# sudo-monkey/fabric-token-sdk

Hardware: AMD Instinct MI355X
Metric: zkatdlog transfer proofs verified/sec (node) + BN254 G1 MSM 2^20 latency (higher is better)
Workload: dtype u32 (Fp/Fr Montgomery); 1 GPU; batch verify 4096 zkatdlog transfers per GPU per step (BASELINE configs[1]); 1-GPU job of 2260992 transfers sharded by tx (configs[3]); batch_per_gpu=4096, device_pass=8192, pp=b=100,e=2, fexp=exact, parallelism=tx-sharded x1

## Files before the change

fabric-token-sdk_amd/csrc/dev/jobs.h:

```cpp
#pragma once
#include "fp29.h"
#include "fp_wide.h"
#include "glv.h"
#include "pairing.h"
#include "sha256.h"

namespace fts {

static constexpr uint32_t NONE = 0xFFFFFFFFu;

struct G1Dev {
  uint32_t x[8], y[8];
};
struct G2Dev {
  uint32_t x0[8], x1[8], y0[8], y1[8];
};
struct F12Dev {
  uint32_t w[96];
};

enum G1Base : uint8_t { G1B_PED0 = 0, G1B_PED1, G1B_PED2, G1B_PEDGEN, G1B_GEN, G1B_COUNT };
static constexpr uint32_t G1B_SIG0 = G1B_COUNT;
static constexpr uint32_t G1B_SIG_MAX_DIGITS = (255 - G1B_SIG0) / 2;
enum G2Base : uint8_t { G2B_PK0 = 0, G2B_PK1, G2B_PK2, G2B_Q, G2B_COUNT };
// ... 27 lines not shown
enum ScalOp : uint32_t { SOP_MUL = 0, SOP_MULK = 1, SOP_SUM = 2, SOP_MADD = 3, SOP_MULK64 = 4 };
struct ScalJob {
  uint32_t op, a, b, out, c;
};

struct VTerm {
  uint32_t pt;
  uint32_t w_lo, w_hi;
  uint32_t flags;
};
static constexpr uint32_t VT_HORNER = 1;
static constexpr uint32_t VT_NEG = 2;

struct G1Job {
  uint32_t fscal[3];
  uint8_t fbase[3];
  uint8_t nfix;
  uint32_t vstart, vcount;
  uint32_t vscal;
  uint32_t vneg;
  uint32_t out;
  uint32_t bytes;
  uint32_t b64;
};

struct G2Job {
  uint32_t fscal[3];
  uint8_t fbase[3];
  uint8_t nfix;
  uint32_t out;
};

struct PairJob {
  uint32_t p1;
  uint32_t p2;
  uint32_t q2;
  uint32_t bytes;
  uint32_t p3;
};

struct Seg {
  uint32_t off, len;
};

struct HashJob {
  uint32_t seg_start, seg_count;
  uint32_t expect;
// ... 607 lines not shown
}

FTS_HD void job_g1(const G1Job& j, const VTerm* vterms, const G1Dev* pts, const uint32_t (*scal)[8],
                   const G1Dev* tab, G1Dev* g1out, uint8_t* arena) {
  g1j acc = jac_inf<fp>();
  if (j.vscal != NONE) {
    g1j V = g1_var_point(j, vterms, pts);
    if (j.vneg) V = jac_neg(V);
    G1Dev loc[16];
    if (!is_zero(V.z)) acc = g1_mul_glv16_iso(g1a{V.x, V.y, false}, V.z, scal[j.vscal], loc, 1);
  }
  for (int f = 0; f < j.nfix; f++) acc = g1_fixed_acc(acc, tab, j.fbase[f], scal[j.fscal[f]]);
  g1a r = jac_to_aff(acc);
  G1Dev d;
  g1_store(d, r);
  g1out[j.out] = d;
  g1_emit_bytes(j, r, arena);
}

FTS_HD void job_g1_part(const G1Job* jobs, uint32_t n, uint32_t i, const VTerm* vterms, const G1Dev* pts,
                        const uint32_t (*scal)[8], const G1Dev* tab, G1JDev* part, G1Dev* vtab) {
  uint32_t f = i / n, jb = i - f * n;
  const G1Job& j = jobs[jb];
  g1j acc = jac_inf<fp>();
  if (f < 3) {
    if (f < j.nfix) acc = g1_fixed_acc(acc, tab, j.fbase[f], scal[j.fscal[f]]);
  } else if (j.vscal != NONE) {
    g1j V = g1_var_point(j, vterms, pts);
    if (j.vneg) V = jac_neg(V);
#if FTS_G1_VAR_W == 16
#if defined(__HIP_DEVICE_COMPILE__)
    G1Dev* tb = vtab + jb;
    const size_t st = n;
#else
    G1Dev loc[16];
    G1Dev* tb = vtab ? vtab + jb : loc;
    const size_t st = vtab ? n : 1;
#endif
    if (!is_zero(V.z)) acc = g1_mul_glv16_iso(g1a{V.x, V.y, false}, V.z, scal[j.vscal], tb, st);
#else
    acc = g1_mul_glv(jac_to_aff(V), scal[j.vscal]);
#endif
  }
  g1j_store(part[i], acc);
}

FTS_HD g1j job_g1_sum_parts(const G1Job& j, uint32_t jb, uint32_t n, const G1JDev* part) {
  g1j acc = g1j_load(part[3 * (size_t)n + jb]);
  for (uint32_t f = 0; f < 3; f++)
    if (f < j.nfix) acc = jac_add(acc, g1j_load(part[(size_t)f * n + jb]));
  return acc;
}

FTS_HD void job_g1_finish(const G1Job& j, const g1j& acc, const fp& zi, G1Dev* g1out, uint8_t* arena) {
  g1a r;
  r.inf = is_zero(acc.z);
  fp zi2 = sqr(zi);
  r.x = r.inf ? fe_zero<ModP>() : acc.x * zi2;
  r.y = r.inf ? fe_zero<ModP>() : acc.y * zi2 * zi;
  G1Dev d;
  g1_store(d, r);
  g1out[j.out] = d;
  g1_emit_bytes(j, r, arena);
}

FTS_HD void g1_pnorm(const g1j& acc, const fp& inv, G1Dev& out) {
  fp z2 = sqr(acc.z);
  G1Dev d;
  g1_store(d, g1a{acc.x * z2 * inv, sqr(z2) * inv, false});
  out = d;
}
// ... 333 lines not shown
```

fabric-token-sdk_amd/csrc/host/planner.cpp:

```cpp
#include "planner.h"

#include <math.h>
#include <string.h>

#include <algorithm>
#include <atomic>
#include <condition_variable>
#include <mutex>
#include <thread>
#include <type_traits>

#include "gojson.h"

namespace ftsh {

static const JField LEAVES_F[] = {{nullptr, JF_STRUCT, nullptr}};
static const JField SIGPROOF_F[] = {{"Signature", JF_STRUCT, LEAVES_F}, {nullptr, JF_STRUCT, nullptr}};
static const JField MP_F[] = {{"SignatureProofs", JF_SLICE, SIGPROOF_F}, {nullptr, JF_STRUCT, nullptr}};
static const JField RANGE_F[] = {{"EqualityProofs", JF_STRUCT, LEAVES_F},
                                 {"MembershipProofs", JF_SLICE, MP_F},
                                 {nullptr, JF_STRUCT, nullptr}};
static const JField RPP_F[] = {{"SignedValues", JF_SLICE, LEAVES_F}, {nullptr, JF_STRUCT, nullptr}};
static const JField PP_F[] = {{"RangeProofParams", JF_STRUCT, RPP_F}, {nullptr, JF_STRUCT, nullptr}};

void Plan::clear() {
  rnd.clear();
  sc1.clear();
  sc_post.clear();
  emit.clear();
  b64.clear();
  cp.clear();
  cp2.clear();
  out.clear();
  out_off.clear();
  item_off.clear();
  dev_pools = false;
  arena_len = out_len = 0;
  wire.clear();
  arena.clear();
  dec.clear();
  zr.clear();
  sc.clear();
  sclist.clear();
  vt.clear();
  g1.clear();
  g1p.clear();
  g2.clear();
  pr.clear();
  seg.clear();
  hpre.clear();
  hmain.clear();
  ck.clear();
  tx.clear();
  n_pts = n_scal = n_g1out = n_g2out = 0;
}

namespace {

// ... 242 lines not shown
    pl.seg.push_back({off, len});
    return (uint32_t)pl.seg.size() - 1;
  }
  uint32_t g1job(std::initializer_list<std::pair<uint8_t, uint32_t>> fixed, const std::vector<VTerm>& var,
                 uint32_t vscal, uint32_t bytes, bool feeds_pairing = false) {
    G1Job j;
    memset(&j, 0, sizeof(j));
    j.nfix = 0;
    for (auto& f : fixed) {
      j.fbase[j.nfix] = f.first;
      j.fscal[j.nfix] = f.second;
      j.nfix++;
    }
    j.vstart = (uint32_t)pl.vt.size();
    j.vcount = (uint32_t)var.size();
    pl.vt.insert(pl.vt.end(), var.begin(), var.end());
    j.vscal = vscal;
    j.vneg = 1;
    j.out = pl.n_g1out++;
    j.bytes = bytes;
    j.b64 = NONE;
    (feeds_pairing ? pl.g1p : pl.g1).push_back(j);
    return j.out;
  }
  uint32_t dbg_scal() { return pp.debug_challenges ? pl.n_scal++ : NONE; }
  static VTerm vterm(uint32_t pt, uint64_t w = 1) {
    VTerm v;
    v.pt = pt;
    v.w_lo = (uint32_t)w;
    v.w_hi = (uint32_t)(w >> 32);
    v.flags = 0;
    return v;
  }

  void begin_tx(uint8_t mode) {
    tc.wf_start = (uint32_t)pl.ck.size();
    ncheck[0] = ncheck[1] = 0;
    part = 0;
    tc.mode = mode;
  }
  void begin_range() {
    tc.wf_count = ncheck[0];
    tc.rg_start = (uint32_t)pl.ck.size();
    part = 1;
  }
  void end_tx() {
// ... 126 lines not shown
  }
  if (s_type == NONE) s_type = scalar(type);
  if (s_sum == NONE) s_sum = scalar(sum);
  if (s_chal == NONE) s_chal = scalar(chal);
  uint32_t s_tn = pl.n_scal++;
  pl.sc.push_back({SOP_MULK, s_type, n, s_tn});
  uint32_t s_bf[64];
  std::vector<uint32_t> bfi(n), vai(n);
  for (uint32_t i = 0; i < n; i++) {
    vai[i] = scalar(vals[i]);
    bfi[i] = scalar(bfs[i]);
  }
  (void)s_bf;
  uint32_t s_bfsum = pl.n_scal++;
  pl.sc.push_back({SOP_SUM, (uint32_t)pl.sclist.size(), n, s_bfsum});
  pl.sclist.insert(pl.sclist.end(), bfi.begin(), bfi.end());
  std::vector<VTerm> all;
  for (uint32_t i = 0; i < n; i++) {
    g1job({{G1B_PED0, s_type}, {G1B_PED1, vai[i]}, {G1B_PED2, bfi[i]}}, {vterm(tok_pt + i)}, s_chal,
          wfout_bytes + 64 * i);
    all.push_back(vterm(tok_pt + i));
  }
  g1job({{G1B_PED0, s_tn}, {G1B_PED1, s_sum}, {G1B_PED2, s_bfsum}}, all, s_chal, wfout_bytes + 64 * n);
  return true;
}

void Builder::decode_range(Doc& doc, RangeDoc& r) {
  int64_t top = doc.top();
  r.chal = doc.elem(doc.f(top, "Challenge"));
  bool isnil;
  int64_t eq = doc.obj(doc.f(top, "EqualityProofs"), isnil);
  r.eq_nil = isnil;
  if (!isnil) {
    r.eq_type = doc.elem(doc.f(eq, "Type"));
    r.eq_val = doc.list(doc.f(eq, "Value"));
    r.eq_tbf = doc.list(doc.f(eq, "TokenBlindingFactor"));
    r.eq_cbf = doc.list(doc.f(eq, "CommitmentBlindingFactor"));
  }
  int64_t mps = doc.f(top, "MembershipProofs");
  if (mps >= 0 && doc.d.at((uint32_t)mps).type != J_NULL) {
    if (doc.d.at((uint32_t)mps).type != J_ARR) {
      doc.err = true;
      return;
    }
    uint32_t n = doc.d.len((uint32_t)mps);
    r.mps.resize(n);
// ... 533 lines not shown
    s.fn = &f;
    s.n = n;
    s.next.store(0);
    s.active = (size_t)nthreads_;
    s.gen++;
  }
  s.cv.notify_all();
  for (size_t i; (i = s.next.fetch_add(1)) < n;) f(i);
  std::unique_lock<std::mutex> lk(s.mu);
  s.done_cv.wait(lk, [&]() { return s.active == 0; });
}

namespace {

constexpr size_t SEC_ALIGN = 256;
constexpr size_t IDX_LIMIT = (size_t)1 << 31;

size_t elem_size(int s) {
  switch (s) {
    case PS_WIRE: case PS_ARENA: case PS_OUT: return 1;
    case PS_DEC: return sizeof(DecodeJob);
    case PS_ZR: return sizeof(ZrJob);
    case PS_SC: case PS_SC1: case PS_SCPOST: return sizeof(ScalJob);
    case PS_SCLIST: return sizeof(uint32_t);
    case PS_VT: return sizeof(VTerm);
    case PS_G1: case PS_G1P: return sizeof(G1Job);
    case PS_G2: return sizeof(G2Job);
    case PS_PR: return sizeof(PairJob);
    case PS_SEG: return sizeof(Seg);
    case PS_HPRE: case PS_HMAIN: return sizeof(HashJob);
    case PS_CK: return sizeof(Check);
    case PS_TX: return sizeof(TxChecks);
    case PS_RND: return sizeof(RandJob);
    case PS_EMIT: return sizeof(EmitJob);
    case PS_B64: return sizeof(B64Job);
    case PS_CP: case PS_CP2: return sizeof(CopyJob);
  }
  return 1;
}

size_t piece_count(const Plan& p, int s) {
  switch (s) {
    case PS_WIRE: return p.wire.size();
    case PS_ARENA: return p.dev_pools ? p.arena_len : p.arena.size();
    case PS_DEC: return p.dec.size();
    case PS_ZR: return p.zr.size();
    case PS_SC: return p.sc.size();
// ... 55 lines not shown
    j.out += o_scal;
    return j;
  };
  const int scs[3] = {PS_SC, PS_SC1, PS_SCPOST};
  const std::vector<ScalJob>* scv[3] = {&b.sc, &b.sc1, &b.sc_post};
  for (int k = 0; k < 3; k++) {
    ScalJob* d = reinterpret_cast<ScalJob*>(dst[scs[k]]) + o.sec[scs[k]];
    for (const ScalJob& j : *scv[k]) *d++ = rel_sc(j);
  }
  uint32_t* sl = reinterpret_cast<uint32_t*>(dst[PS_SCLIST]) + o.sec[PS_SCLIST];
  for (uint32_t v : b.sclist) *sl++ = v + o_scal;
  VTerm* vt = reinterpret_cast<VTerm*>(dst[PS_VT]) + o.sec[PS_VT];
  for (VTerm v : b.vt) {
    v.pt += o_pts;
    *vt++ = v;
  }
  for (int side = 0; side < 2; side++) {
    int sec = side ? PS_G1P : PS_G1;
    G1Job* d = reinterpret_cast<G1Job*>(dst[sec]) + o.sec[sec];
    for (G1Job j : (side ? b.g1p : b.g1)) {
      for (int k = 0; k < j.nfix; k++) j.fscal[k] += o_scal;
      j.vstart += o_vt;
      j.vscal = rel(j.vscal, o_scal);
      j.out += o_g1;
      j.bytes = rel(j.bytes, o_arena);
      j.b64 = rel(j.b64, o_arena);
      *d++ = j;
    }
  }
  G2Job* g2 = reinterpret_cast<G2Job*>(dst[PS_G2]) + o.sec[PS_G2];
  for (G2Job j : b.g2) {
    for (int k = 0; k < j.nfix; k++) j.fscal[k] += o_scal;
    j.out += o_g2;
    *g2++ = j;
  }
  PairJob* pr = reinterpret_cast<PairJob*>(dst[PS_PR]) + o.sec[PS_PR];
  for (PairJob j : b.pr) {
    j.p1 += o_g1;
    j.p2 += p2_g1out ? o_g1 : o_pts;
    j.q2 = rel(j.q2, o_g2);
    j.p3 = rel(j.p3, o_g1);
    j.bytes += o_arena;
    *pr++ = j;
  }
  Seg* sg = reinterpret_cast<Seg*>(dst[PS_SEG]) + o.sec[PS_SEG];
  for (Seg s : b.seg) {
// ... 42 lines not shown
  }
  B64Job* bj = reinterpret_cast<B64Job*>(dst[PS_B64]) + o.sec[PS_B64];
  for (B64Job j : b.b64) {
    j.src += o_arena;
    j.dst += o_out;
    *bj++ = j;
  }
  const int cps[2] = {PS_CP, PS_CP2};
  const std::vector<CopyJob>* cpv[2] = {&b.cp, &b.cp2};
  for (int k = 0; k < 2; k++) {
    CopyJob* d = reinterpret_cast<CopyJob*>(dst[cps[k]]) + o.sec[cps[k]];
    for (CopyJob j : *cpv[k]) {
      j.src += o_wire;
      j.dst += j.to_out ? o_out : o_arena;
      *d++ = j;
    }
  }
}

void relocate_piece(const Plan& b, const PieceBase& o, const FlatPlan& fp, uint8_t* blob) {
  uint8_t* dst[PS_COUNT];
  for (int s = 0; s < PS_COUNT; s++) dst[s] = blob + fp.off[s];
  relocate_into(b, o, fp.p2_g1out, false, dst);
}

}

std::string flat_layout(const PlanWork& w, bool p2_g1out, FlatPlan& fp) {
  fp.p2_g1out = p2_g1out;
  fp.base.assign(w.used, PieceBase{});
  fp.out_off.clear();
  fp.item_off.clear();
  fp.n_items = 0;
  size_t cur[PS_COUNT] = {};
  cur[PS_ARENA] = C_SIZE;
  uint64_t pts = 0, scal = 0, g1 = 0, g2 = 0;
  for (size_t k = 0; k < w.used; k++) {
    const Plan& p = w.pieces[k];
    PieceBase& b = fp.base[k];
    cur[PS_WIRE] = (cur[PS_WIRE] + 15) & ~(size_t)15;
    cur[PS_ARENA] = (cur[PS_ARENA] + 15) & ~(size_t)15;
    for (int s = 0; s < PS_COUNT; s++) {
      b.sec[s] = cur[s];
      cur[s] += piece_count(p, s);
    }
    b.pts = (uint32_t)pts;
    b.scal = (uint32_t)scal;
    b.g1out = (uint32_t)g1;
    b.g2out = (uint32_t)g2;
    pts += p.n_pts;
    scal += p.n_scal;
    g1 += p.n_g1out;
    g2 += p.n_g2out;
    for (uint32_t v : p.out_off) fp.out_off.push_back((uint32_t)(v + b.sec[PS_OUT]));
    for (uint32_t v : p.item_off) fp.item_off.push_back((uint32_t)(v + b.sec[PS_ARENA]));
    fp.n_items += p.tx.size();
  }
  if (!fp.out_off.empty() || cur[PS_OUT]) fp.out_off.push_back((uint32_t)cur[PS_OUT]);
  for (int s = 0; s < PS_COUNT; s++)
    if (cur[s] >= IDX_LIMIT) return "batch too large for 32-bit job indices (split it into smaller batches)";
  if (pts >= IDX_LIMIT || scal >= IDX_LIMIT || g1 >= IDX_LIMIT || g2 >= IDX_LIMIT)
    return "batch too large for 32-bit job indices (split it into smaller batches)";
  fp.n_pts = (uint32_t)pts;
  fp.n_scal = (uint32_t)scal;
  fp.n_g1out = (uint32_t)g1;
  fp.n_g2out = (uint32_t)g2;
  fp.dev_pools = w.used > 0;
  for (size_t k = 0; k < w.used; k++) fp.dev_pools = fp.dev_pools && w.pieces[k].dev_pools;
  int order[PS_COUNT], no = 0;
  for (int s = 0; s < PS_COUNT; s++)
    if (!fp.dev_pools || (s != PS_ARENA && s != PS_OUT)) order[no++] = s;
  if (fp.dev_pools) {
    order[no++] = PS_ARENA;
    order[no++] = PS_OUT;
  }
  size_t off = 0;
  for (int q = 0; q < PS_COUNT; q++) {
    int s = order[q];
    if (fp.dev_pools && s == PS_ARENA) fp.upload = off;
    fp.cnt[s] = cur[s];
    fp.off[s] = off;
    size_t bytes = cur[s] * elem_size(s) + (s == PS_WIRE ? WIRE_TAIL : 0);
    off = (off + bytes + SEC_ALIGN - 1) & ~(SEC_ALIGN - 1);
  }
// ... 87 lines not shown
  take(out.arena, PS_ARENA);
  take(out.dec, PS_DEC);
  take(out.zr, PS_ZR);
  take(out.sc, PS_SC);
  take(out.sclist, PS_SCLIST);
  take(out.vt, PS_VT);
  take(out.g1, PS_G1);
  take(out.g1p, PS_G1P);
  take(out.g2, PS_G2);
  take(out.pr, PS_PR);
  take(out.seg, PS_SEG);
  take(out.hpre, PS_HPRE);
  take(out.hmain, PS_HMAIN);
  take(out.ck, PS_CK);
  take(out.tx, PS_TX);
  take(out.rnd, PS_RND);
  take(out.sc1, PS_SC1);
  take(out.sc_post, PS_SCPOST);
  take(out.emit, PS_EMIT);
  take(out.b64, PS_B64);
  take(out.cp, PS_CP);
  take(out.cp2, PS_CP2);
  take(out.out, PS_OUT);
  out.out_off = fp.out_off;
  out.item_off = fp.item_off;
  out.p2_g1out = fp.p2_g1out;
  out.n_pts = fp.n_pts;
  out.n_scal = fp.n_scal;
  out.n_g1out = fp.n_g1out;
  out.n_g2out = fp.n_g2out;
}

size_t plan_piece_count(size_t n, int threads) {
  return std::max<size_t>(1, std::min<size_t>((size_t)std::max(1, threads), n / 32));
}

void plan_items(const PPInfo& pp, size_t n, const PlanItem* items, PlanWork& w, WorkPool& pool) {
  size_t np = plan_piece_count(n, pool.size());
  if (w.pieces.size() < np) w.pieces.resize(np);
  w.used = np;
  pool.run(np, [&](size_t c) {
    Plan& p = w.pieces[c];
    p.clear();
    size_t lo = n * c / np, hi = n * (c + 1) / np;
    Builder b(p, pp);
    for (size_t i = lo; i < hi; i++) {
// ... 297 lines not shown
```

fabric-token-sdk_amd/csrc/host/planner.h:

```cpp
#pragma once
#include <stdint.h>

#include <functional>
#include <string>
#include <vector>

#include "../dev/jobs.h"

namespace ftsh {

using namespace fts;

enum : uint32_t {
  C_PEDGEN = 0,
  C_PED0 = 64,
  C_PED1 = 128,
  C_PED2 = 192,
  C_Q_PK = 256,
  C_PK_Q = 384,
  C_SIZE = 896,
};
static constexpr uint32_t CONST_FLAG = 0x80000000u;

struct PPInfo {
// ... 27 lines not shown
  std::vector<DecodeJob> dec;
  std::vector<ZrJob> zr;
  std::vector<ScalJob> sc;
  std::vector<uint32_t> sclist;
  std::vector<VTerm> vt;
  std::vector<G1Job> g1;
  std::vector<G1Job> g1p;
  std::vector<G2Job> g2;
  std::vector<PairJob> pr;
  std::vector<Seg> seg;
  std::vector<HashJob> hpre, hmain;
  std::vector<Check> ck;
  std::vector<TxChecks> tx;
  std::vector<RandJob> rnd;
  std::vector<ScalJob> sc1;
  std::vector<ScalJob> sc_post;
  std::vector<EmitJob> emit;
  std::vector<B64Job> b64;
  std::vector<CopyJob> cp;
  std::vector<CopyJob> cp2;
  std::vector<uint8_t> out;
  std::vector<uint32_t> out_off;
  std::vector<uint32_t> item_off;
  bool p2_g1out = false;
  bool dev_pools = false;
  size_t arena_len = 0, out_len = 0;
  uint32_t n_pts = 0, n_scal = 0, n_g1out = 0, n_g2out = 0;
  void clear();
};

struct TransferIn {
  const uint8_t* inputs;
  uint32_t n_in;
  const uint8_t* outputs;
  uint32_t n_out;
  const uint8_t* proof;
  size_t proof_len;
};
struct IssueIn {
  const uint8_t* outputs;
  uint32_t n_out;
  const uint8_t* proof;
  size_t proof_len;
  uint8_t anonymous;
};

// ... 9 lines not shown
  uint8_t kind;
  TransferIn t;
  IssueIn i;
  OpeningIn o;
};

class WorkPool {
 public:
  explicit WorkPool(int threads);
  ~WorkPool();
  WorkPool(const WorkPool&) = delete;
  WorkPool& operator=(const WorkPool&) = delete;
  void run(size_t n, const std::function<void(size_t)>& f);
  int size() const { return nthreads_ + 1; }

 private:
  struct State;
  State* st_;
  int nthreads_;
};

enum PlanSec : int {
  PS_WIRE, PS_ARENA, PS_DEC, PS_ZR, PS_SC, PS_SCLIST, PS_VT, PS_G1, PS_G1P, PS_G2, PS_PR, PS_SEG, PS_HPRE,
  PS_HMAIN, PS_CK, PS_TX, PS_RND, PS_SC1, PS_SCPOST, PS_EMIT, PS_B64, PS_CP, PS_CP2, PS_OUT, PS_COUNT
};
static constexpr size_t WIRE_TAIL = 64;

struct PieceBase {
  size_t sec[PS_COUNT];
  uint32_t pts, scal, g1out, g2out;
};

struct FlatPlan {
  size_t off[PS_COUNT] = {};
  size_t cnt[PS_COUNT] = {};
  size_t bytes = 0;
  size_t upload = 0;
  bool dev_pools = false;
  size_t n_items = 0;
  uint32_t n_pts = 0, n_scal = 0, n_g1out = 0, n_g2out = 0;
  bool p2_g1out = false;
  std::vector<PieceBase> base;
  std::vector<uint32_t> out_off;
  std::vector<uint32_t> item_off;
  template <class T>
  T* ptr(uint8_t* blob, PlanSec s) const { return reinterpret_cast<T*>(blob + off[s]); }
};

struct PlanWork {
  std::vector<Plan> pieces;
  std::vector<std::string> errs;
  size_t used = 0;
};

size_t plan_piece_count(size_t n, int threads);
void plan_items(const PPInfo& pp, size_t n, const PlanItem* items, PlanWork& w, WorkPool& pool);
std::string flat_layout(const PlanWork& w, bool p2_g1out, FlatPlan& fp);
void flat_write(const PlanWork& w, const FlatPlan& fp, uint8_t* blob, const uint8_t* const_bytes, WorkPool& pool);

void plan_transfers(const PPInfo& pp, size_t n, const TransferIn* tx, Plan& out, int threads);
void plan_issues(const PPInfo& pp, size_t n, const IssueIn* is, Plan& out, int threads);
void plan_unflatten(const FlatPlan& fp, const uint8_t* blob, Plan& out);
PieceBase plan_append(Plan& d, const Plan& b);
void plan_items_merged(const PPInfo& pp, size_t n, const PlanItem* items, Plan& out, int threads);

struct TransferWit {
  const uint8_t* inputs;
  uint32_t n_in;
  const uint8_t* outputs;
  uint32_t n_out;
  const uint8_t* in_values;
// ... 25 lines not shown
```

fabric-token-sdk_amd/csrc/k_g1.hip:

```cpp
#include <hip/hip_runtime.h>

#include "dev/binv.h"
#include "dev/jobs.h"
#include "launch.h"

#ifndef FTS_G1PART_PRIO
#define FTS_G1PART_PRIO 0
#endif
#ifndef FTS_COMBINE_PRIO
#define FTS_COMBINE_PRIO FTS_BINV_PRIO
#endif

using namespace fts;

#define JOB_KERNEL_PROLOGUE(n)                          \
  uint32_t i = blockIdx.x * blockDim.x + threadIdx.x; \
  if (i >= (n)) return;

__global__ void __launch_bounds__(128) k_g1_part(const G1Job* jobs, uint32_t n, const VTerm* vt, const G1Dev* pts,
                                                 const uint32_t (*scal)[8], const G1Dev* tab, G1JDev* part,
                                                 G1Dev* vtab) {
  uint32_t i = blockIdx.x * blockDim.x + threadIdx.x;
  if (i >= 4 * n) return;
#if FTS_G1PART_PRIO
  __builtin_amdgcn_s_setprio(FTS_G1PART_PRIO);
#endif
  job_g1_part(jobs, n, i, vt, pts, scal, tab, part, vtab);
}

template <int NT>
__device__ fp block_batch_inv(fp x, uint32_t (*pre)[NT], uint32_t (*suf)[NT], uint32_t* tot) {
  const int t = threadIdx.x;
  if (is_zero(x)) x = fe_one<ModP>();
  fp p = x, q = x;
#pragma unroll
  for (int k = 0; k < 8; k++) {
    pre[k][t] = p.v[k];
    suf[k][t] = q.v[k];
  }
  __syncthreads();
#pragma nounroll
  for (int off = 1; off < NT; off <<= 1) {
    fp a = fe_one<ModP>(), b = fe_one<ModP>();
    if (t >= off)
#pragma unroll
      for (int k = 0; k < 8; k++) a.v[k] = pre[k][t - off];
// ... 100 lines not shown
```

fabric-token-sdk_amd/csrc/launch.h:

```cpp
#pragma once
#include <hip/hip_runtime.h>

#include "dev/jobs.h"
#include "dev/msm.h"
#include "dev/idemix.h"
#include "dev/sx29.h"

using namespace fts;

static constexpr uint32_t SX_JOBS_PER_WAVE = 10;
struct SyncWave {
  __device__ __forceinline__ void operator()() const { __syncthreads(); }
};
#define SX_SLOTS_DECL(NS)                                                          \
  static constexpr uint32_t sx_stride_ = (NS) * (sizeof(F2Slot) / 16) + 1;          \
  __shared__ uint4 sx_raw_[SX_JOBS_PER_WAVE * sx_stride_];
#define SX_KERNEL_PROLOGUE(n)                                           \
  uint32_t lane_ = threadIdx.x, sx_ = lane_ / 6;                        \
  bool ghost_ = sx_ >= SX_JOBS_PER_WAVE;                                \
  int k_ = ghost_ ? (int)(lane_ - 6 * SX_JOBS_PER_WAVE) : (int)(lane_ - 6 * sx_); \
  if (ghost_) sx_ = SX_JOBS_PER_WAVE - 1;                               \
  uint32_t job_ = blockIdx.x * SX_JOBS_PER_WAVE + sx_;                  \
  bool valid = !ghost_ && job_ < (n);                                   \
  uint32_t jc = job_ < (n) ? job_ : (n) - 1;                            \
// ... 2 lines not shown
#define SQ_KERNEL_PROLOGUE(n, NS) SQ_KERNEL_PROLOGUE_B(n, NS, SX_B)
#define SQ_KERNEL_PROLOGUE_B(n, NS, BOFS)                                         \
  static constexpr uint32_t sq_stride_ = sq_region_dwords(NS) / 2;               \
  __shared__ uint2 sq_raw_[SX_JOBS_PER_WAVE * sq_stride_];                       \
  uint32_t lane_ = threadIdx.x, sx_ = lane_ / 6;                                 \
  bool ghost_ = sx_ >= SX_JOBS_PER_WAVE;                                         \
  int k_ = ghost_ ? (int)(lane_ - 6 * SX_JOBS_PER_WAVE) : (int)(lane_ - 6 * sx_); \
  if (ghost_) sx_ = SX_JOBS_PER_WAVE - 1;                                        \
  uint32_t job_ = blockIdx.x * SX_JOBS_PER_WAVE + sx_;                           \
  bool valid = !ghost_ && job_ < (n);                                            \
  uint32_t jc = job_ < (n) ? job_ : (n) - 1;                                     \
  Sq<SyncWave, BOFS> x{k_, (QSlotT*)(sq_raw_ + sx_ * sq_stride_), !ghost_, {}};

__global__ void k_decode(const DecodeJob* jobs, uint32_t n, const uint8_t* wire, G1Dev* pts, uint8_t* pt_ok,
                         uint8_t* arena);
__global__ void k_zr(const ZrJob* jobs, uint32_t n, const uint8_t* wire, uint32_t (*scal)[8], uint8_t* canon);
__global__ void k_scalar(const ScalJob* jobs, uint32_t n, uint32_t (*scal)[8], const uint32_t* list);
__global__ void k_hash(const HashJob* jobs, uint32_t n, const Seg* segs, const uint8_t* arena, uint32_t (*scal)[8],
                       const uint8_t* canon, uint8_t* ok);
__global__ void k_verdict(const TxChecks* tx, uint32_t n, const Check* ck, const uint8_t* pt_ok,
                          const uint8_t* hash_ok, int32_t* codes, uint32_t* bitmap);
__global__ void k_pp_decode(const uint8_t* raw, const uint32_t* g1off, uint32_t n1, const uint32_t* g2off,
                            uint32_t n2, G1Dev* g1, G2Dev* g2, uint8_t* g1bytes, uint8_t* g2bytes, uint8_t* ok);
__global__ void k_g1_part(const G1Job* jobs, uint32_t n, const VTerm* vt, const G1Dev* pts,
                          const uint32_t (*scal)[8], const G1Dev* tab, G1JDev* part, G1Dev* vtab);
__global__ void k_g1_combine(const G1Job* jobs, uint32_t n, const G1JDev* part, G1Dev* g1out, uint8_t* arena,
                             G1Dev* pnorm);
__global__ void k_tab_g1(const G1Dev* bases, uint32_t n, G1Dev* tab);
__global__ void k_tab_g1_bw(const G1Dev* bases, uint32_t nb, G1Dev* bw);
__global__ void k_tab_g1_fill(const G1Dev* bw, uint32_t nb, uint32_t chunk, G1JDev* jtmp, uint32_t (*zs)[8], G1Dev* tab);
__global__ void k_g2(const G2Job* jobs, uint32_t n, const uint32_t (*scal)[8], const G2Dev* tab, G2Dev* g2out);
__global__ void k_g2lines(const G2Job* g2, const PairJob* pr, uint32_t n, const uint32_t (*scal)[8], const G2Dev* tab,
                          G2Dev* g2out, const G1Dev* pts, EvLineDev* lines);
__global__ void k_g2_part(const G2Job* g2, uint32_t n, const uint32_t (*scal)[8], const G2Dev* tab, G2PartDev* part);
#ifndef FTS_G2LINES_X29
#define FTS_G2LINES_X29 1
#endif
#ifndef FTS_G2_BINV
#define FTS_G2_BINV 1
#endif
__global__ void k_g2_sum(uint32_t n, G2PartDev* part);
__global__ void k_g2_binv(uint32_t n, G2PartDev* part);
__global__ void k_g2lines1(const G2Job* g2, const PairJob* pr, uint32_t n, const G2PartDev* part, G2Dev* g2out,
                           const G1Dev* pts, EvLineDev* lines);
__global__ void k_tab_g2(const G2Dev* bases, uint32_t n, G2Dev* tab);
__global__ void k_tab_g2_bw(const G2Dev* bases, G2Dev* bw);
__global__ void k_tab_g2_fill(const G2Dev* bw, uint32_t chunk, uint32_t (*jt)[48], uint32_t (*zs)[16], G2Dev* tab);
__global__ void k_miller(const PairJob* jobs, uint32_t n, const LineCoef29* qlines, const EvLineDev* lines2,
// ... 92 lines not shown
```

fabric-token-sdk_amd/csrc/runtime.hip:

```cpp
#include <hip/hip_runtime.h>

#include <chrono>
#include <stdio.h>
#include <stdlib.h>
#include <string.h>

#include <algorithm>
#include <mutex>
#include <string>
#include <thread>
#include <vector>

#include "../../include/ftsamd.h"
#include "dev/jobs.h"
#include "host/planner.h"
#include "launch.h"

using namespace fts;
using namespace ftsh;

#include "rt_internal.h"

thread_local std::string g_err;
int set_err(int code, const std::string& msg) {
// ... 486 lines not shown

static const G1Dev* prover_g1tab(ftz_ctx* c) { return c->ptab_ready ? c->g1tab_p.p : c->g1tab.p; }

int prover_plan(ftz_batch* b, size_t n, const void* wit, int kind) {
  ftz_ctx* c = b->ctx;
  int trc = ensure_prover_tables(c);
  if (trc != FTZ_SUCCESS) return trc;
  const PPInfo& pp = c->ptab_ready ? c->pp : c->pp_var;
  std::string e = kind == 0
                      ? plan_prove_items_transfers(pp, n, static_cast<const TransferWit*>(wit), b->work, *c->pool)
                      : plan_prove_items_issues(pp, n, static_cast<const IssueWit*>(wit), b->work, *c->pool);
  if (!e.empty()) return set_err(FTZ_E_INVALID, e);
  return slot_finish_plan(b, n, true);
}

struct SlotPtrs {
  uint8_t *wire, *arena, *out;
  const DecodeJob* dec;
  const ZrJob* zr;
  const ScalJob *sc, *sc1, *sc_post;
  const uint32_t* sclist;
  const VTerm* vt;
  const G1Job *g1, *g1p;
  const G2Job* g2;
  const PairJob* pr;
  const Seg* seg;
  const HashJob *hpre, *hmain;
  const Check* ck;
  const TxChecks* tx;
  const RandJob* rnd;
  const EmitJob* emit;
  const B64Job* b64;
  const CopyJob *cp, *cp2;
  G1Dev* pts;
  uint8_t *pt_ok, *canon, *hash_ok, *hash_ok_pre;
  uint32_t (*scal)[8];
  G1Dev* g1out;
  G1Dev* pnorm;
  G2Dev* g2out;
  F12Dev* fbuf;
  int32_t* fxpark;
  EvLineDev* lines2;
  G1JDev *part1, *part1p;
  G2PartDev* part2;
  G1Dev *vtab1, *vtab1p;
  int32_t* codes;
  uint32_t* bitmap;
  uint32_t n_dec, n_zr, n_sc, n_sc1, n_sp, n_rnd, n_em, n_b64, n_g1, n_g1p, n_g2, n_pr, n_hp, n_hm, n_tx, n_cp, n_cp2;
};

static SlotPtrs slot_ptrs(ftz_batch* b) {
  SlotPtrs p;
  const FlatPlan& f = b->fp;
  uint8_t* d = b->d_blob.p;
  uint8_t* s = b->d_scr.p;
  p.wire = d + f.off[PS_WIRE];
  p.arena = d + f.off[PS_ARENA];
  p.out = d + f.off[PS_OUT];
  p.dec = f.ptr<DecodeJob>(d, PS_DEC);
  p.zr = f.ptr<ZrJob>(d, PS_ZR);
  p.sc = f.ptr<ScalJob>(d, PS_SC);
  p.sc1 = f.ptr<ScalJob>(d, PS_SC1);
  p.sc_post = f.ptr<ScalJob>(d, PS_SCPOST);
  p.sclist = f.ptr<uint32_t>(d, PS_SCLIST);
  p.vt = f.ptr<VTerm>(d, PS_VT);
  p.g1 = f.ptr<G1Job>(d, PS_G1);
  p.g1p = f.ptr<G1Job>(d, PS_G1P);
  p.g2 = f.ptr<G2Job>(d, PS_G2);
  p.pr = f.ptr<PairJob>(d, PS_PR);
  p.seg = f.ptr<Seg>(d, PS_SEG);
  p.hpre = f.ptr<HashJob>(d, PS_HPRE);
  p.hmain = f.ptr<HashJob>(d, PS_HMAIN);
  p.ck = f.ptr<Check>(d, PS_CK);
  p.tx = f.ptr<TxChecks>(d, PS_TX);
  p.rnd = f.ptr<RandJob>(d, PS_RND);
  p.emit = f.ptr<EmitJob>(d, PS_EMIT);
  p.b64 = f.ptr<B64Job>(d, PS_B64);
  p.cp = f.ptr<CopyJob>(d, PS_CP);
  p.cp2 = f.ptr<CopyJob>(d, PS_CP2);
  const ScratchLayout& l = b->sl;
  p.pts = reinterpret_cast<G1Dev*>(s + l.pts);
  p.pt_ok = s + l.pt_ok;
  p.scal = reinterpret_cast<uint32_t (*)[8]>(s + l.scal);
  p.canon = s + l.canon;
  p.g1out = reinterpret_cast<G1Dev*>(s + l.g1out);
  p.pnorm = reinterpret_cast<G1Dev*>(s + l.pnorm);
  p.g2out = reinterpret_cast<G2Dev*>(s + l.g2out);
  p.fbuf = reinterpret_cast<F12Dev*>(s + l.fbuf);
  p.fxpark = reinterpret_cast<int32_t*>(s + l.fxpark);
  p.lines2 = reinterpret_cast<EvLineDev*>(s + l.lines2);
  p.part1 = reinterpret_cast<G1JDev*>(s + l.part1);
  p.part1p = reinterpret_cast<G1JDev*>(s + l.part1p);
  p.part2 = reinterpret_cast<G2PartDev*>(s + l.part2);
  p.vtab1 = reinterpret_cast<G1Dev*>(s + l.vtab1);
  p.vtab1p = reinterpret_cast<G1Dev*>(s + l.vtab1p);
  p.hash_ok = s + l.hash_ok;
  p.hash_ok_pre = s + l.hash_ok_pre;
  p.codes = reinterpret_cast<int32_t*>(s + l.codes);
  p.bitmap = reinterpret_cast<uint32_t*>(s + l.bitmap);
  p.n_dec = (uint32_t)f.cnt[PS_DEC];
  p.n_zr = (uint32_t)f.cnt[PS_ZR];
  p.n_sc = (uint32_t)f.cnt[PS_SC];
  p.n_sc1 = (uint32_t)f.cnt[PS_SC1];
  p.n_sp = (uint32_t)f.cnt[PS_SCPOST];
  p.n_rnd = (uint32_t)f.cnt[PS_RND];
  p.n_em = (uint32_t)f.cnt[PS_EMIT];
  p.n_b64 = (uint32_t)f.cnt[PS_B64];
  p.n_g1 = (uint32_t)f.cnt[PS_G1];
  p.n_g1p = (uint32_t)f.cnt[PS_G1P];
  p.n_g2 = (uint32_t)f.cnt[PS_G2];
  p.n_pr = (uint32_t)f.cnt[PS_PR];
  p.n_hp = (uint32_t)f.cnt[PS_HPRE];
  p.n_hm = (uint32_t)f.cnt[PS_HMAIN];
  p.n_tx = (uint32_t)f.cnt[PS_TX];
  p.n_cp = (uint32_t)f.cnt[PS_CP];
  p.n_cp2 = (uint32_t)f.cnt[PS_CP2];
  return p;
}

static hipError_t upload_plan(ftz_batch* b, hipStream_t s) {
  const FlatPlan& f = b->fp;
  hipError_t e = hipMemcpyAsync(b->d_blob.p, b->h_blob.p, f.upload, hipMemcpyHostToDevice, s);
  if (e == hipSuccess && f.dev_pools)
    e = hipMemcpyAsync(b->d_blob.p + f.off[PS_ARENA], b->h_blob.p + f.off[PS_ARENA], C_SIZE, hipMemcpyHostToDevice, s);
  return e;
}

static void launch_g2lines(ftz_ctx* c, const SlotPtrs& p, const G1Dev* pts, hipStream_t s, bool prover) {
  int layout = prover ? c->g2lanes_prover : c->g2lanes;
  if (!prover && !c->g2lanes_set && p.n_g2 <= c->opt.small_pass) layout = FTZ_LAYOUT_SEXTET;
  if (layout == FTZ_LAYOUT_ONE_LANE) {
    k_g2_part<<<blocks_for(4 * p.n_g2, 64), 64, 0, s>>>(p.g2, p.n_g2, p.scal, c->g2tab.p, p.part2);
#if FTS_G2_BINV && FTS_G2LINES_X29
    k_g2_sum<<<blocks_for(p.n_g2, 64), 64, 0, s>>>(p.n_g2, p.part2);
    k_g2_binv<<<blocks_for(p.n_g2, 256), 256, 0, s>>>(p.n_g2, p.part2);
#endif
    k_g2lines1<<<blocks_for(p.n_g2, 64), 64, 0, s>>>(p.g2, p.pr, p.n_g2, p.part2, p.g2out, pts, p.lines2);
  } else {
    k_g2lines<<<blocks_for(p.n_g2, SX_JOBS_PER_WAVE), 64, 0, s>>>(p.g2, p.pr, p.n_g2, p.scal, c->g2tab.p, p.g2out, pts,
                                                                  p.lines2);
  }
}

static void launch_miller(ftz_ctx* c, const SlotPtrs& p, hipStream_t s) {
  if (c->qnorm) {
    k_miller_n<<<blocks_for(p.n_pr, SX_JOBS_PER_WAVE), 64, 0, s>>>(p.pr, p.n_pr, c->qlines29n.p, p.lines2, p.g1out,
                                                                   p.pnorm, p.fbuf);
    return;
// ... 19 lines not shown
  HC(hipEventRecord(e[18], s));
  if (upload) HC(upload_plan(b, s));
  HC(hipMemsetAsync(p.bitmap, 0, sizeof(uint32_t) * ((b->n + 31) / 32 + 1), s));
  if (b->fp.n_pts) HC(hipMemsetAsync(p.pt_ok, 1, b->fp.n_pts, s));
  HC(hipEventRecord(e[0], s));
  if (p.n_cp) k_copy<<<p.n_cp, 64, 0, s>>>(p.cp, p.n_cp, p.wire, p.arena, p.out);
  if (p.n_cp2) k_copy<<<p.n_cp2, 64, 0, s>>>(p.cp2, p.n_cp2, p.wire, p.arena, p.out);
  if (p.n_dec) k_decode<<<blocks_for(p.n_dec, 256), 256, 0, s>>>(p.dec, p.n_dec, p.wire, p.pts, p.pt_ok, p.arena);
  HC(hipEventRecord(e[1], s));
  if (p.n_zr) k_zr<<<blocks_for(p.n_zr, 256), 256, 0, s>>>(p.zr, p.n_zr, p.wire, p.scal, p.canon);
  HC(hipEventRecord(e[2], s));
  if (p.n_hp)
    k_hash<<<blocks_for(p.n_hp, 128), 128, 0, s>>>(p.hpre, p.n_hp, p.seg, p.arena, p.scal, p.canon, p.hash_ok_pre);
  HC(hipEventRecord(e[3], s));
  if (p.n_sc) k_scalar<<<blocks_for(p.n_sc, 256), 256, 0, s>>>(p.sc, p.n_sc, p.scal, p.sclist);
  HC(hipEventRecord(e[4], s));
  HC(hipStreamWaitEvent(s3, e[4], 0));
  HC(hipEventRecord(e[14], s3));
  if (p.n_g2)
    launch_g2lines(c, p, p.pts, s3, false);
  HC(hipEventRecord(e[15], s3));
  HC(hipEventRecord(e[16], s));
  if (p.n_g1p) {
    k_g1_part<<<blocks_for(4 * p.n_g1p, 128), 128, 0, s>>>(p.g1p, p.n_g1p, p.vt, p.pts, p.scal, c->g1tab.p, p.part1p,
                                                           p.vtab1p);
    k_g1_combine<<<blocks_for(p.n_g1p, 256), 256, 0, s>>>(p.g1p, p.n_g1p, p.part1p, p.g1out, p.arena, p.pnorm);
  }
  HC(hipEventRecord(e[5], s));
  HC(hipStreamWaitEvent(s2, e[4], 0));
  HC(hipEventRecord(e[11], s2));
  if (p.n_g1) {
    k_g1_part<<<blocks_for(4 * p.n_g1, 128), 128, 0, s2>>>(p.g1, p.n_g1, p.vt, p.pts, p.scal, c->g1tab.p, p.part1,
                                                           p.vtab1);
    k_g1_combine<<<blocks_for(p.n_g1, 256), 256, 0, s2>>>(p.g1, p.n_g1, p.part1, p.g1out, p.arena, p.pnorm);
  }
  HC(hipEventRecord(e[12], s2));
  HC(hipStreamWaitEvent(s, e[15], 0));
  HC(hipEventRecord(e[6], s));
  if (p.n_pr)
    launch_miller(c, p, s);
  HC(hipEventRecord(e[7], s));
  launch_fexp(c, p, s);
  HC(hipEventRecord(e[8], s));
  HC(hipStreamWaitEvent(s, e[12], 0));
  HC(hipEventRecord(e[9], s));
  if (p.n_hm)
    k_hash<<<blocks_for(p.n_hm, 128), 128, 0, s>>>(p.hmain, p.n_hm, p.seg, p.arena, p.scal, p.canon, p.hash_ok);
  HC(hipEventRecord(e[10], s));
  if (p.n_tx)
    k_verdict<<<blocks_for(p.n_tx, 256), 256, 0, s>>>(p.tx, p.n_tx, p.ck, p.pt_ok, p.hash_ok, p.codes, p.bitmap);
  HC(hipEventRecord(e[13], s));
  if (fetch_codes && b->n) HC(hipMemcpyAsync(b->h_res.p, p.codes, b->n * sizeof(int32_t), hipMemcpyDeviceToHost, s));
  HC(hipEventRecord(e[17], s));
  HC(hipGetLastError());
  b->pending = true;
  return FTZ_SUCCESS;
}
// ... 172 lines not shown
  for (int k = 0; k < FTZ_NKERNELS; k++) b->jobs_last[k] = jobs[k];
  hipEvent_t* e = b->ev;
  HC(hipEventRecord(e[18], s));
  if (upload) HC(upload_plan(b, s));
  HC(hipMemsetAsync(p.bitmap, 0, sizeof(uint32_t) * ((b->n + 31) / 32 + 1), s));
  if (b->fp.n_pts) HC(hipMemsetAsync(p.pt_ok, 1, b->fp.n_pts, s));
  HC(hipEventRecord(e[0], s));
  if (p.n_cp) k_copy<<<p.n_cp, 64, 0, s>>>(p.cp, p.n_cp, p.wire, p.arena, p.out);
  if (p.n_cp2) k_copy<<<p.n_cp2, 64, 0, s>>>(p.cp2, p.n_cp2, p.wire, p.arena, p.out);
  if (p.n_dec) k_decode<<<blocks_for(p.n_dec, 256), 256, 0, s>>>(p.dec, p.n_dec, p.wire, p.pts, p.pt_ok, p.arena);
  HC(hipEventRecord(e[1], s));
  if (p.n_zr) k_zr<<<blocks_for(p.n_zr, 256), 256, 0, s>>>(p.zr, p.n_zr, p.wire, p.scal, p.canon);
  HC(hipEventRecord(e[2], s));
  if (p.n_rnd) k_rand<<<blocks_for(p.n_rnd, 128), 128, 0, s>>>(p.rnd, p.n_rnd, p.arena, p.scal);
  if (p.n_hp)
    k_hash<<<blocks_for(p.n_hp, 128), 128, 0, s>>>(p.hpre, p.n_hp, p.seg, p.arena, p.scal, p.canon, p.hash_ok_pre);
  HC(hipEventRecord(e[3], s));
  if (p.n_sc) k_scalar<<<blocks_for(p.n_sc, 256), 256, 0, s>>>(p.sc, p.n_sc, p.scal, p.sclist);
  if (p.n_sc1) k_scalar<<<blocks_for(p.n_sc1, 256), 256, 0, s>>>(p.sc1, p.n_sc1, p.scal, p.sclist);
  HC(hipEventRecord(e[4], s));
  HC(hipStreamWaitEvent(s2, e[4], 0));
  HC(hipEventRecord(e[11], s2));
  if (p.n_g1) {
    k_g1_part<<<blocks_for(4 * p.n_g1, 128), 128, 0, s2>>>(p.g1, p.n_g1, p.vt, p.pts, p.scal, prover_g1tab(c), p.part1,
                                                           p.vtab1);
    k_g1_combine<<<blocks_for(p.n_g1, 256), 256, 0, s2>>>(p.g1, p.n_g1, p.part1, p.g1out, p.arena, p.pnorm);
  }
  HC(hipEventRecord(e[12], s2));
  HC(hipEventRecord(e[16], s));
  if (p.n_g1p) {
    k_g1_part<<<blocks_for(4 * p.n_g1p, 128), 128, 0, s>>>(p.g1p, p.n_g1p, p.vt, p.pts, p.scal, prover_g1tab(c), p.part1p,
                                                           p.vtab1p);
    k_g1_combine<<<blocks_for(p.n_g1p, 256), 256, 0, s>>>(p.g1p, p.n_g1p, p.part1p, p.g1out, p.arena, p.pnorm);
  }
  HC(hipEventRecord(e[5], s));
  HC(hipStreamWaitEvent(s3, e[5], 0));
  HC(hipEventRecord(e[14], s3));
  if (p.n_g2)
    launch_g2lines(c, p, p.g1out, s3, true);
  HC(hipEventRecord(e[15], s3));
  HC(hipStreamWaitEvent(s, e[15], 0));
  HC(hipEventRecord(e[6], s));
  if (p.n_pr && p.n_g2 == 0 && c->pp.fixed_pairs && c->ptab_ready)
    k_miller_f3<<<blocks_for(p.n_pr, SX_JOBS_PER_WAVE), 64, 0, s>>>(p.pr, p.n_pr, c->qlines29n.p, c->pklines29n.p,
                                                                    p.g1out, p.pnorm, p.fbuf);
  else if (p.n_pr)
    launch_miller(c, p, s);
  HC(hipEventRecord(e[7], s));
  launch_fexp(c, p, s);
  HC(hipEventRecord(e[8], s));
  HC(hipStreamWaitEvent(s, e[12], 0));
  HC(hipEventRecord(e[9], s));
  if (p.n_hm)
    k_hash<<<blocks_for(p.n_hm, 128), 128, 0, s>>>(p.hmain, p.n_hm, p.seg, p.arena, p.scal, p.canon, p.hash_ok);
  if (p.n_sp) k_scalar<<<blocks_for(p.n_sp, 256), 256, 0, s>>>(p.sc_post, p.n_sp, p.scal, p.sclist);
  HC(hipEventRecord(e[10], s));
// ... 312 lines not shown
```

Measured before the change: 904,400 transfers/s.

## Share per-token variable-base G1 chains with sum job and compact part lanes

Measured after the change: 924,700 transfers/s, median of 6. 1.02x the previous value.

```diff
diff --git a/fabric-token-sdk_amd/csrc/dev/jobs.h b/fabric-token-sdk_amd/csrc/dev/jobs.h
--- a/fabric-token-sdk_amd/csrc/dev/jobs.h
+++ b/fabric-token-sdk_amd/csrc/dev/jobs.h
@@ -73,7 +73,10 @@
   uint32_t out;
   uint32_t bytes;
   uint32_t b64;
-};
+  uint32_t sh_first, sh_count;
+};
+static constexpr uint32_t G1_SHARE_MAX = 8;
+FTS_HD bool g1_own_chain(const G1Job& j) { return j.vscal != NONE && j.sh_count == 0; }
 
 struct G2Job {
   uint32_t fscal[3];
@@ -727,6 +730,7 @@
                         const uint32_t (*scal)[8], const G1Dev* tab, G1JDev* part, G1Dev* vtab) {
   uint32_t f = i / n, jb = i - f * n;
   const G1Job& j = jobs[jb];
+  if (f == 3 && j.sh_count) return;
   g1j acc = jac_inf<fp>();
   if (f < 3) {
     if (f < j.nfix) acc = g1_fixed_acc(acc, tab, j.fbase[f], scal[j.fscal[f]]);
@@ -751,7 +755,13 @@
 }
 
 FTS_HD g1j job_g1_sum_parts(const G1Job& j, uint32_t jb, uint32_t n, const G1JDev* part) {
-  g1j acc = g1j_load(part[3 * (size_t)n + jb]);
+  g1j acc = jac_inf<fp>();
+  if (j.sh_count) {
+    acc = g1j_load(part[3 * (size_t)n + j.sh_first]);
+    for (uint32_t s = 1; s < j.sh_count; s++) acc = jac_add(acc, g1j_load(part[3 * (size_t)n + j.sh_first + s]));
+  } else if (j.vscal != NONE) {
+    acc = g1j_load(part[3 * (size_t)n + jb]);
+  }
   for (uint32_t f = 0; f < 3; f++)
     if (f < j.nfix) acc = jac_add(acc, g1j_load(part[(size_t)f * n + jb]));
   return acc;
diff --git a/fabric-token-sdk_amd/csrc/host/planner.cpp b/fabric-token-sdk_amd/csrc/host/planner.cpp
--- a/fabric-token-sdk_amd/csrc/host/planner.cpp
+++ b/fabric-token-sdk_amd/csrc/host/planner.cpp
@@ -34,6 +34,10 @@
   out.clear();
   out_off.clear();
   item_off.clear();
+  g1fl.clear();
+  g1vl.clear();
+  g1pfl.clear();
+  g1pvl.clear();
   dev_pools = false;
   arena_len = out_len = 0;
   wire.clear();
@@ -322,6 +326,20 @@
     j.b64 = NONE;
     (feeds_pairing ? pl.g1p : pl.g1).push_back(j);
     return j.out;
+  }
+  void share_var(std::vector<G1Job>& jobs, uint32_t count) {
+    if (count == 0 || count > G1_SHARE_MAX || jobs.size() < (size_t)count + 1) return;
+    G1Job& j = jobs.back();
+    const uint32_t first = (uint32_t)(jobs.size() - 1 - count);
+    if (j.vscal == NONE || j.vcount != count) return;
+    for (uint32_t s = 0; s < count; s++) {
+      const G1Job& q = jobs[first + s];
+      if (q.vscal != j.vscal || q.vneg != j.vneg || q.vcount != 1 || q.sh_count) return;
+      const VTerm &a = pl.vt[j.vstart + s], &b = pl.vt[q.vstart];
+      if (a.pt != b.pt || a.flags || b.flags || vterm_w(a) != 1 || vterm_w(b) != 1) return;
+    }
+    j.sh_first = first;
+    j.sh_count = count;
   }
   uint32_t dbg_scal() { return pp.debug_challenges ? pl.n_scal++ : NONE; }
   static VTerm vterm(uint32_t pt, uint64_t w = 1) {
@@ -494,6 +512,7 @@
     all.push_back(vterm(tok_pt + i));
   }
   g1job({{G1B_PED0, s_tn}, {G1B_PED1, s_sum}, {G1B_PED2, s_bfsum}}, all, s_chal, wfout_bytes + 64 * n);
+  share_var(pl.g1, n);
   return true;
 }
 
@@ -1073,7 +1092,7 @@
     case PS_DEC: return sizeof(DecodeJob);
     case PS_ZR: return sizeof(ZrJob);
     case PS_SC: case PS_SC1: case PS_SCPOST: return sizeof(ScalJob);
-    case PS_SCLIST: return sizeof(uint32_t);
+    case PS_SCLIST: case PS_G1FL: case PS_G1VL: case PS_G1PFL: case PS_G1PVL: return sizeof(uint32_t);
     case PS_VT: return sizeof(VTerm);
     case PS_G1: case PS_G1P: return sizeof(G1Job);
     case PS_G2: return sizeof(G2Job);
@@ -1175,6 +1194,7 @@
       for (int k = 0; k < j.nfix; k++) j.fscal[k] += o_scal;
       j.vstart += o_vt;
       j.vscal = rel(j.vscal, o_scal);
+      if (j.sh_count) j.sh_first += (uint32_t)o.sec[sec];
       j.out += o_g1;
       j.bytes = rel(j.bytes, o_arena);
       j.b64 = rel(j.b64, o_arena);
@@ -1263,8 +1283,30 @@
   uint8_t* dst[PS_COUNT];
   for (int s = 0; s < PS_COUNT; s++) dst[s] = blob + fp.off[s];
   relocate_into(b, o, fp.p2_g1out, false, dst);
-}
-
+  for (int side = 0; side < 2; side++) {
+    const int sec = side ? PS_G1P : PS_G1, fl = side ? PS_G1PFL : PS_G1FL, vl = side ? PS_G1PVL : PS_G1VL;
+    const std::vector<G1Job>& jobs = side ? b.g1p : b.g1;
+    g1_part_lists(jobs.data(), jobs.size(), o.sec[sec], fp.cnt[sec], reinterpret_cast<uint32_t*>(dst[fl]) + o.sec[fl],
+                  reinterpret_cast<uint32_t*>(dst[vl]) + o.sec[vl]);
+  }
+}
+
+}
+
+void g1_list_counts(const std::vector<G1Job>& jobs, size_t& nf, size_t& nv) {
+  nf = nv = 0;
+  for (const G1Job& j : jobs) {
+    nf += j.nfix;
+    nv += g1_own_chain(j);
+  }
+}
+
+void g1_part_lists(const G1Job* jobs, size_t cnt, size_t base, size_t n, uint32_t* fixed, uint32_t* var) {
+  for (uint32_t f = 0; f < 3; f++)
+    for (size_t k = 0; k < cnt; k++)
+      if (f < jobs[k].nfix) *fixed++ = (uint32_t)(f * n + base + k);
+  for (size_t k = 0; k < cnt; k++)
+    if (g1_own_chain(jobs[k])) *var++ = (uint32_t)(3 * n + base + k);
 }
 
 std::string flat_layout(const PlanWork& w, bool p2_g1out, FlatPlan& fp) {
@@ -1285,6 +1327,13 @@
       b.sec[s] = cur[s];
       cur[s] += piece_count(p, s);
     }
+    size_t nf, nv;
+    g1_list_counts(p.g1, nf, nv);
+    cur[PS_G1FL] += nf;
+    cur[PS_G1VL] += nv;
+    g1_list_counts(p.g1p, nf, nv);
+    cur[PS_G1PFL] += nf;
+    cur[PS_G1PVL] += nv;
     b.pts = (uint32_t)pts;
     b.scal = (uint32_t)scal;
     b.g1out = (uint32_t)g1;
@@ -1301,6 +1350,8 @@
   for (int s = 0; s < PS_COUNT; s++)
     if (cur[s] >= IDX_LIMIT) return "batch too large for 32-bit job indices (split it into smaller batches)";
   if (pts >= IDX_LIMIT || scal >= IDX_LIMIT || g1 >= IDX_LIMIT || g2 >= IDX_LIMIT)
+    return "batch too large for 32-bit job indices (split it into smaller batches)";
+  if (cur[PS_G1] >= IDX_LIMIT / 2 || cur[PS_G1P] >= IDX_LIMIT / 2)
     return "batch too large for 32-bit job indices (split it into smaller batches)";
   fp.n_pts = (uint32_t)pts;
   fp.n_scal = (uint32_t)scal;
@@ -1434,6 +1485,10 @@
   take(out.cp, PS_CP);
   take(out.cp2, PS_CP2);
   take(out.out, PS_OUT);
+  take(out.g1fl, PS_G1FL);
+  take(out.g1vl, PS_G1VL);
+  take(out.g1pfl, PS_G1PFL);
+  take(out.g1pvl, PS_G1PVL);
   out.out_off = fp.out_off;
   out.item_off = fp.item_off;
   out.p2_g1out = fp.p2_g1out;
diff --git a/fabric-token-sdk_amd/csrc/host/planner.h b/fabric-token-sdk_amd/csrc/host/planner.h
--- a/fabric-token-sdk_amd/csrc/host/planner.h
+++ b/fabric-token-sdk_amd/csrc/host/planner.h
@@ -73,6 +73,7 @@
   std::vector<uint8_t> out;
   std::vector<uint32_t> out_off;
   std::vector<uint32_t> item_off;
+  std::vector<uint32_t> g1fl, g1vl, g1pfl, g1pvl;
   bool p2_g1out = false;
   bool dev_pools = false;
   size_t arena_len = 0, out_len = 0;
@@ -128,7 +129,8 @@
 
 enum PlanSec : int {
   PS_WIRE, PS_ARENA, PS_DEC, PS_ZR, PS_SC, PS_SCLIST, PS_VT, PS_G1, PS_G1P, PS_G2, PS_PR, PS_SEG, PS_HPRE,
-  PS_HMAIN, PS_CK, PS_TX, PS_RND, PS_SC1, PS_SCPOST, PS_EMIT, PS_B64, PS_CP, PS_CP2, PS_OUT, PS_COUNT
+  PS_HMAIN, PS_CK, PS_TX, PS_RND, PS_SC1, PS_SCPOST, PS_EMIT, PS_B64, PS_CP, PS_CP2, PS_OUT,
+  PS_G1FL, PS_G1VL, PS_G1PFL, PS_G1PVL, PS_COUNT
 };
 static constexpr size_t WIRE_TAIL = 64;
 
@@ -153,6 +155,9 @@
   T* ptr(uint8_t* blob, PlanSec s) const { return reinterpret_cast<T*>(blob + off[s]); }
 };
 
+void g1_list_counts(const std::vector<G1Job>& jobs, size_t& nf, size_t& nv);
+void g1_part_lists(const G1Job* jobs, size_t cnt, size_t base, size_t n, uint32_t* fixed, uint32_t* var);
+
 struct PlanWork {
   std::vector<Plan> pieces;
   std::vector<std::string> errs;
diff --git a/fabric-token-sdk_amd/csrc/k_g1.hip b/fabric-token-sdk_amd/csrc/k_g1.hip
--- a/fabric-token-sdk_amd/csrc/k_g1.hip
+++ b/fabric-token-sdk_amd/csrc/k_g1.hip
@@ -17,11 +17,19 @@
   uint32_t i = blockIdx.x * blockDim.x + threadIdx.x; \
   if (i >= (n)) return;
 
-__global__ void __launch_bounds__(128) k_g1_part(const G1Job* jobs, uint32_t n, const VTerm* vt, const G1Dev* pts,
-                                                 const uint32_t (*scal)[8], const G1Dev* tab, G1JDev* part,
-                                                 G1Dev* vtab) {
-  uint32_t i = blockIdx.x * blockDim.x + threadIdx.x;
-  if (i >= 4 * n) return;
+__global__ void __launch_bounds__(128) k_g1_part(const G1Job* jobs, uint32_t n, const uint32_t* flist, uint32_t nfl,
+                                                 const uint32_t* vlist, uint32_t nvl, const VTerm* vt,
+                                                 const G1Dev* pts, const uint32_t (*scal)[8], const G1Dev* tab,
+                                                 G1JDev* part, G1Dev* vtab) {
+  const uint32_t lane = blockIdx.x * blockDim.x + threadIdx.x, vbase = (nfl + 63) & ~63u;
+  uint32_t i;
+  if (lane < vbase) {
+    if (lane >= nfl) return;
+    i = flist[lane];
+  } else {
+    if (lane - vbase >= nvl) return;
+    i = vlist[lane - vbase];
+  }
 #if FTS_G1PART_PRIO
   __builtin_amdgcn_s_setprio(FTS_G1PART_PRIO);
 #endif
diff --git a/fabric-token-sdk_amd/csrc/launch.h b/fabric-token-sdk_amd/csrc/launch.h
--- a/fabric-token-sdk_amd/csrc/launch.h
+++ b/fabric-token-sdk_amd/csrc/launch.h
@@ -48,8 +48,10 @@
                           const uint8_t* hash_ok, int32_t* codes, uint32_t* bitmap);
 __global__ void k_pp_decode(const uint8_t* raw, const uint32_t* g1off, uint32_t n1, const uint32_t* g2off,
                             uint32_t n2, G1Dev* g1, G2Dev* g2, uint8_t* g1bytes, uint8_t* g2bytes, uint8_t* ok);
-__global__ void k_g1_part(const G1Job* jobs, uint32_t n, const VTerm* vt, const G1Dev* pts,
-                          const uint32_t (*scal)[8], const G1Dev* tab, G1JDev* part, G1Dev* vtab);
+__global__ void k_g1_part(const G1Job* jobs, uint32_t n, const uint32_t* flist, uint32_t nfl, const uint32_t* vlist,
+                          uint32_t nvl, const VTerm* vt, const G1Dev* pts, const uint32_t (*scal)[8], const G1Dev* tab,
+                          G1JDev* part, G1Dev* vtab);
+static inline uint32_t g1_part_lanes(uint32_t nfl, uint32_t nvl) { return ((nfl + 63) & ~63u) + nvl; }
 __global__ void k_g1_combine(const G1Job* jobs, uint32_t n, const G1JDev* part, G1Dev* g1out, uint8_t* arena,
                              G1Dev* pnorm);
 __global__ void k_tab_g1(const G1Dev* bases, uint32_t n, G1Dev* tab);
diff --git a/fabric-token-sdk_amd/csrc/runtime.hip b/fabric-token-sdk_amd/csrc/runtime.hip
--- a/fabric-token-sdk_amd/csrc/runtime.hip
+++ b/fabric-token-sdk_amd/csrc/runtime.hip
@@ -532,6 +532,7 @@
   const uint32_t* sclist;
   const VTerm* vt;
   const G1Job *g1, *g1p;
+  const uint32_t *g1fl, *g1vl, *g1pfl, *g1pvl;
   const G2Job* g2;
   const PairJob* pr;
   const Seg* seg;
@@ -557,6 +558,7 @@
   int32_t* codes;
   uint32_t* bitmap;
   uint32_t n_dec, n_zr, n_sc, n_sc1, n_sp, n_rnd, n_em, n_b64, n_g1, n_g1p, n_g2, n_pr, n_hp, n_hm, n_tx, n_cp, n_cp2;
+  uint32_t n_g1fl, n_g1vl, n_g1pfl, n_g1pvl;
 };
 
 static SlotPtrs slot_ptrs(ftz_batch* b) {
@@ -576,6 +578,10 @@
   p.vt = f.ptr<VTerm>(d, PS_VT);
   p.g1 = f.ptr<G1Job>(d, PS_G1);
   p.g1p = f.ptr<G1Job>(d, PS_G1P);
+  p.g1fl = f.ptr<uint32_t>(d, PS_G1FL);
+  p.g1vl = f.ptr<uint32_t>(d, PS_G1VL);
+  p.g1pfl = f.ptr<uint32_t>(d, PS_G1PFL);
+  p.g1pvl = f.ptr<uint32_t>(d, PS_G1PVL);
   p.g2 = f.ptr<G2Job>(d, PS_G2);
   p.pr = f.ptr<PairJob>(d, PS_PR);
   p.seg = f.ptr<Seg>(d, PS_SEG);
@@ -618,6 +624,10 @@
   p.n_b64 = (uint32_t)f.cnt[PS_B64];
   p.n_g1 = (uint32_t)f.cnt[PS_G1];
   p.n_g1p = (uint32_t)f.cnt[PS_G1P];
+  p.n_g1fl = (uint32_t)f.cnt[PS_G1FL];
+  p.n_g1vl = (uint32_t)f.cnt[PS_G1VL];
+  p.n_g1pfl = (uint32_t)f.cnt[PS_G1PFL];
+  p.n_g1pvl = (uint32_t)f.cnt[PS_G1PVL];
   p.n_g2 = (uint32_t)f.cnt[PS_G2];
   p.n_pr = (uint32_t)f.cnt[PS_PR];
   p.n_hp = (uint32_t)f.cnt[PS_HPRE];
@@ -634,6 +644,18 @@
   if (e == hipSuccess && f.dev_pools)
     e = hipMemcpyAsync(b->d_blob.p + f.off[PS_ARENA], b->h_blob.p + f.off[PS_ARENA], C_SIZE, hipMemcpyHostToDevice, s);
   return e;
+}
+
+static void launch_g1(const SlotPtrs& p, bool pairing, const G1Dev* tab, hipStream_t s) {
+  const G1Job* jobs = pairing ? p.g1p : p.g1;
+  const uint32_t n = pairing ? p.n_g1p : p.n_g1;
+  const uint32_t nfl = pairing ? p.n_g1pfl : p.n_g1fl, nvl = pairing ? p.n_g1pvl : p.n_g1vl;
+  G1JDev* part = pairing ? p.part1p : p.part1;
+  if (const uint32_t lanes = g1_part_lanes(nfl, nvl))
+    k_g1_part<<<blocks_for(lanes, 128), 128, 0, s>>>(jobs, n, pairing ? p.g1pfl : p.g1fl, nfl,
+                                                     pairing ? p.g1pvl : p.g1vl, nvl, p.vt, p.pts, p.scal, tab, part,
+                                                     pairing ? p.vtab1p : p.vtab1);
+  k_g1_combine<<<blocks_for(n, 256), 256, 0, s>>>(jobs, n, part, p.g1out, p.arena, p.pnorm);
 }
 
 static void launch_g2lines(ftz_ctx* c, const SlotPtrs& p, const G1Dev* pts, hipStream_t s, bool prover) {
@@ -699,17 +721,13 @@
   HC(hipEventRecord(e[15], s3));
   HC(hipEventRecord(e[16], s));
   if (p.n_g1p) {
-    k_g1_part<<<blocks_for(4 * p.n_g1p, 128), 128, 0, s>>>(p.g1p, p.n_g1p, p.vt, p.pts, p.scal, c->g1tab.p, p.part1p,
-                                                           p.vtab1p);
-    k_g1_combine<<<blocks_for(p.n_g1p, 256), 256, 0, s>>>(p.g1p, p.n_g1p, p.part1p, p.g1out, p.arena, p.pnorm);
+    launch_g1(p, true, c->g1tab.p, s);
   }
   HC(hipEventRecord(e[5], s));
   HC(hipStreamWaitEvent(s2, e[4], 0));
   HC(hipEventRecord(e[11], s2));
   if (p.n_g1) {
-    k_g1_part<<<blocks_for(4 * p.n_g1, 128), 128, 0, s2>>>(p.g1, p.n_g1, p.vt, p.pts, p.scal, c->g1tab.p, p.part1,
-                                                           p.vtab1);
-    k_g1_combine<<<blocks_for(p.n_g1, 256), 256, 0, s2>>>(p.g1, p.n_g1, p.part1, p.g1out, p.arena, p.pnorm);
+    launch_g1(p, false, c->g1tab.p, s2);
   }
   HC(hipEventRecord(e[12], s2));
   HC(hipStreamWaitEvent(s, e[15], 0));
@@ -928,16 +946,12 @@
   HC(hipStreamWaitEvent(s2, e[4], 0));
   HC(hipEventRecord(e[11], s2));
   if (p.n_g1) {
-    k_g1_part<<<blocks_for(4 * p.n_g1, 128), 128, 0, s2>>>(p.g1, p.n_g1, p.vt, p.pts, p.scal, prover_g1tab(c), p.part1,
-                                                           p.vtab1);
-    k_g1_combine<<<blocks_for(p.n_g1, 256), 256, 0, s2>>>(p.g1, p.n_g1, p.part1, p.g1out, p.arena, p.pnorm);
+    launch_g1(p, false, prover_g1tab(c), s2);
   }
   HC(hipEventRecord(e[12], s2));
   HC(hipEventRecord(e[16], s));
   if (p.n_g1p) {
-    k_g1_part<<<blocks_for(4 * p.n_g1p, 128), 128, 0, s>>>(p.g1p, p.n_g1p, p.vt, p.pts, p.scal, prover_g1tab(c), p.part1p,
-                                                           p.vtab1p);
-    k_g1_combine<<<blocks_for(p.n_g1p, 256), 256, 0, s>>>(p.g1p, p.n_g1p, p.part1p, p.g1out, p.arena, p.pnorm);
+    launch_g1(p, true, prover_g1tab(c), s);
   }
   HC(hipEventRecord(e[5], s));
   HC(hipStreamWaitEvent(s3, e[5], 0));
```
